# XiaoshuiHuang/IMFNet

Hardware: AMD Instinct MI355X
Metric: descriptors/sec (32-D) on 3DMatch fragments (higher is better)
Workload: dtype f32 (bf16x3)

## Files before the change

### imfnet_amd/_lib.py

```python
import ctypes as C
import os

_HERE = os.path.dirname(os.path.abspath(__file__))
LIB_PATH = os.environ.get("IMF_LIB") or os.path.join(_HERE, "libimfnet_hip.so")

TILE_ROWS = 64
MASK_WORDS = 4
MAX_KVOL = 125
MAX_BATCH = 8
FLAG_RANGE = 32
XYZ_F32_QUOTIENT = 2
TAG_LABEL, TAG_REGS, TAG_WAVE8, TAG_WAVE4, TAG_HEAD, TAG_HALF, TAG_U48, TAG_OCC = 1, 2, 4, 8, 16, 64, 128, 256


class ImfError(RuntimeError):
    pass


class ConvArgs(C.Structure):
    _fields_ = [
        ("in_a", C.c_void_p), ("in_b", C.c_void_p),
        ("c_a", C.c_int32), ("c_b", C.c_int32),
        ("w_packed", C.c_void_p),
        ("kvol", C.c_int32), ("cout", C.c_int32),
        ("tile_rows", C.c_void_p), ("nbr", C.c_void_p),
        ("tile_mask", C.c_void_p),
        ("n_slots", C.c_int64), ("n_out", C.c_int64),
        ("scale", C.c_void_p), ("shift", C.c_void_p), ("residual", C.c_void_p),
        ("relu", C.c_int32), ("l2norm", C.c_int32),
        ("out", C.c_void_p),
        ("split_k", C.c_int32), ("variant", C.c_int32),
        ("workspace", C.c_void_p), ("workspace_bytes", C.c_size_t),
        ("ev_begin", C.c_void_p), ("ev_end", C.c_void_p),
        ("n_out_dev", C.c_void_p), ("slots_extra", C.c_int32),
        ("kernel_tag", C.c_int32), ("dyn_err", C.c_void_p), ("geglu", C.c_int32), ("operand_format", C.c_int32),
    ]


class HeadArgs(C.Structure):
    _fields_ = [
        ("in_a", C.c_void_p), ("in_b", C.c_void_p), ("c_a", C.c_int32), ("c_b", C.c_int32),
        ("w1_packed", C.c_void_p), ("scale1", C.c_void_p), ("shift1", C.c_void_p),
        ("relu1", C.c_int32), ("c_mid", C.c_int32),
        ("w2_packed", C.c_void_p), ("scale2", C.c_void_p), ("shift2", C.c_void_p),
        ("l2norm", C.c_int32), ("c_out", C.c_int32),
        ("n", C.c_int64), ("n_dev", C.c_void_p), ("out", C.c_void_p), ("flags", C.c_void_p),
        ("ev_begin", C.c_void_p), ("ev_end", C.c_void_p), ("a_split", C.c_int32), ("variant", C.c_int32),
    ]


class LevelDesc(C.Structure):
    _fields_ = [("coords", C.c_void_p), ("table", C.c_void_p),
                ("capacity", C.c_int64), ("first_idx", C.c_void_p), ("cap_rows", C.c_int64),
                ("tensor_stride", C.c_int32)]


class FusionWeights(C.Structure):
    _fields_ = [(n, C.c_void_p) for n in ("ln1_g", "ln1_b", "wq_p", "wo_p", "bo", "ln2_g", "ln2_b", "w1_p", "b1",
                                          "w2_p", "b2", "w1_f32", "w2_f32")]


class NetConv(C.Structure):
    _fields_ = [("w_packed", C.c_void_p), ("kvol", C.c_int32), ("cin", C.c_int32), ("cout", C.c_int32),
                ("scale", C.c_void_p), ("shift", C.c_void_p), ("relu", C.c_int32), ("l2norm", C.c_int32),
                ("variant", C.c_int32)]


class ResunetDesc(C.Structure):
    _fields_ = [("channels", C.c_int32 * 5), ("tr_channels", C.c_int32 * 5), ("in_channels", C.c_int32),
                ("out_channels", C.c_int32), ("first_ksize", C.c_int32), ("small_first", C.c_int32),
                ("conv", NetConv * 23), ("first_kernel", C.c_void_p), ("first_scale", C.c_void_p),
                ("first_shift", C.c_void_p), ("fusion", FusionWeights), ("fusion_scale", C.c_float),
                ("first_kernel_image", C.c_void_p)]


class ImageDesc(C.Structure):
    _fields_ = [("stem_w", C.c_void_p), ("stem_scale", C.c_void_p), ("stem_shift", C.c_void_p),
                ("conv", NetConv * 15), ("ln_g", C.c_void_p), ("ln_b", C.c_void_p), ("kv_w", C.c_void_p),
                ("variant", C.c_int32)]


class ImageTable(C.Structure):
    _fields_ = [("tile_rows", C.c_void_p), ("nbr", C.c_void_p), ("tile_mask", C.c_void_p), ("n_slots", C.c_int64),
                ("n_out", C.c_int64), ("kvol", C.c_int32)]


IMAGE_TRAIN_TABLES = ("t4", "t48", "t48T", "td", "tdT", "t8")


class ImageTrainTables(C.Structure):
    _fields_ = [(n, ImageTable) for n in IMAGE_TRAIN_TABLES]


class NetTrace(C.Structure):
    _fields_ = [("ev_begin", C.c_void_p), ("ev_end", C.c_void_p), ("nbr", C.c_void_p), ("kvol", C.c_int32),
                ("cin", C.c_int32), ("cout", C.c_int32), ("split", C.c_int32), ("n_slots", C.c_int64),
                ("n_out", C.c_int64), ("launched", C.c_int32), ("level", C.c_int32), ("slots_extra", C.c_int32),
                ("kernel_tag", C.c_int32)]


class ResunetIO(C.Structure):
    _fields_ = [("level", LevelDesc * 4), ("n", C.c_int64 * 4), ("bbox", C.c_void_p), ("x", C.c_void_p),
                ("x_all_ones", C.c_int32), ("n_items", C.c_int32), ("item_row0", C.c_int64 * MAX_BATCH),
                ("item_rows", C.c_int64 * MAX_BATCH), ("kt_packed", C.c_void_p * MAX_BATCH),
                ("v_packed", C.c_void_p * MAX_BATCH),
                ("n_tokens", C.c_int32), ("tokens_padded", C.c_int32), ("image_ready", C.c_void_p),
                ("fusion_done", C.c_void_p), ("int_arena", C.c_void_p), ("int_arena_bytes", C.c_size_t),
                ("float_arena", C.c_void_p), ("float_arena_bytes", C.c_size_t), ("out", C.c_void_p),
                ("events", C.c_void_p * 16), ("side_stream", C.c_void_p), ("main_stream", C.c_void_p),
                ("trace", C.POINTER(NetTrace)), ("dyn", C.c_int32), ("meta", C.c_void_p),
                ("bitgrid_words", C.c_size_t), ("pyramid", C.c_void_p), ("flags", C.c_void_p),
                ("fp32_buffers", C.c_int32)]


DYN_WORDS = 16
META_WORDS = 64


class FragmentCaps(C.Structure):
    _fields_ = [("n_points", C.c_int64), ("rows", C.c_int64 * 4), ("n_items", C.c_int32), ("img_h", C.c_int32),
                ("img_w", C.c_int32), ("bitgrid_words", C.c_size_t)]


class FragmentIO(C.Structure):
    _fields_ = [("xyz", C.c_void_p), ("xyz_is_f64", C.c_int32), ("voxel_size", C.c_double), ("dyn", C.c_void_p),
                ("image", C.c_void_p), ("meta", C.c_void_p), ("pyramid_arena", C.c_void_p),
                ("pyramid_arena_bytes", C.c_size_t), ("image_ws", C.c_void_p), ("image_ws_bytes", C.c_size_t),
                ("kt_packed", C.c_void_p), ("v_packed", C.c_void_p), ("tokens_padded", C.c_int32),
                ("int_arena", C.c_void_p), ("int_arena_bytes", C.c_size_t), ("float_arena", C.c_void_p),
                ("float_arena_bytes", C.c_size_t), ("out", C.c_void_p), ("events", C.c_void_p * 16),
                ("main_stream", C.c_void_p), ("side_stream", C.c_void_p), ("image_stream", C.c_void_p),
                ("trace", C.POINTER(NetTrace)), ("levels", LevelDesc * 4), ("serialize", C.c_int32),
                ("fp32_buffers", C.c_int32), ("head_on_side", C.c_int32), ("gpu_idle_hint", C.c_int32),
                ("inputs_event", C.c_void_p), ("reuse_event", C.c_void_p)]


class TsdfParams(C.Structure):
    _fields_ = [("fx", C.c_double), ("fy", C.c_double), ("cx", C.c_double), ("cy", C.c_double),
                ("voxel_length", C.c_double), ("sdf_trunc", C.c_double), ("depth_scale", C.c_double),
                ("depth_trunc", C.c_double), ("lattice_offset", C.c_double), ("height", C.c_int32), ("width", C.c_int32)]


class OverlapIndex(C.Structure):
    _fields_ = [("table", C.c_void_p), ("capacity", C.c_int64), ("xyz", C.c_void_p), ("idx", C.c_void_p),
                ("cells", C.c_void_p), ("chunks", C.c_void_p), ("meta", C.c_void_p), ("n", C.c_int64), ("cell", C.c_double)]


class Job(C.Structure):
    _fields_ = [("net", C.POINTER(ResunetDesc)), ("img", C.POINTER(ImageDesc)), ("caps", C.POINTER(FragmentCaps)),
                ("io", C.POINTER(FragmentIO)), ("host_in", C.c_void_p), ("dev_in", C.c_void_p), ("in_bytes", C.c_size_t),
                ("dev_out", C.c_void_p), ("host_out", C.c_void_p), ("out_bytes", C.c_size_t), ("sel", C.c_void_p),
                ("sel_offset", C.c_size_t), ("out_offset", C.c_size_t), ("out_row_bytes", C.c_int32),
                ("defer_download", C.c_int32)]


PIPELINE_SDMA_COPIES = 1

_P, _I, _L, _D, _Z = C.c_void_p, C.c_int, C.c_int64, C.c_double, C.c_size_t

SIGNATURES = {
    "imf_version": (_I, []),
    "imf_last_error": (C.c_char_p, []),
    "imf_spconv_wgrad_workspace_bytes": (_Z, [_L, _I, _I, _I]),
    "imf_spconv_wgrad": (_I, [_P, _I, _P, _I, _P, _P, _L, _L, _I, _P, _P, _Z, _P]),
    "imf_bn_train_chunk_rows": (_I, []),
    "imf_bn_train_workspace_bytes": (_Z, [_L, _I]),
    "imf_bn_train_forward": (_I, [_P, _L, _I, _P, _P, _D, _P, _I, _P, _P, _D, _P, _P, _P, _Z, _P]),
    "imf_bn_train_backward": (_I, [_P, _P, _P, _I, _P, _P, _L, _I, _P, _P, _P, _P, _P, _Z, _P]),
    "imf_hc_loss_workspace_bytes": (_Z, [_L, _L, _I, _L, _L, _L, _L]),
    "imf_hc_loss_forward": (_I, [_P, _L, _P, _L, _I, _P, _L, _P, _L, _P, _L, _P, _L, _D, _D, _P, _P, _P, _P, _P, _P, _P,
                                 _Z, _P]),
    "imf_hc_loss_backward": (_I, [_P, _L, _P, _L, _I, _P, _L, _P, _L, _P, _L, _P, _L, _D, _D, _P, _P, _P, _P, _P, _P, _P,
                                  _P, _P, _Z, _P]),
    "imf_fusion_train_chunk_rows": (_I, []),
    "imf_fusion_train_saved_bytes": (_Z, [_L, _I, _I]),
    "imf_fusion_train_workspace_bytes": (_Z, [_L, _I, _I]),
    "imf_fusion_train_forward": (_I, [_P, _L, _P, _I, _P, _I, _I, _I, _I, _I, C.POINTER(C.c_void_p), _P, _P, _Z, _P, _P]),
    "imf_fusion_train_backward": (_I, [_P, _P, _L, _P, _I, _P, _I, _I, _I, _I, _I, C.POINTER(C.c_void_p), _P, _Z, _P, _P,
                                       C.POINTER(C.c_void_p), _P, _P, _Z, _P]),
    "imf_dam_heat": (_I, [_P, _L, _P, _P, _I, _I, _P, _I, _I, _P, _P, _P, _P, _P]),
    "imf_ply_vertex_count": (_L, [C.c_char_p]),
    "imf_ply_read_points": (_L, [C.c_char_p, _P, _L]),
    "imf_png_info": (_I, [C.c_char_p, C.POINTER(C.c_int), C.POINTER(C.c_int), C.POINTER(C.c_int)]),
    "imf_png_read_f32": (_I, [C.c_char_p, _P, _L, C.POINTER(C.c_int), C.POINTER(C.c_int), C.POINTER(C.c_int)]),
    "imf_png_read_u16": (_I, [C.c_char_p, _P, _L, C.POINTER(C.c_int), C.POINTER(C.c_int)]),
    "imf_ply_write_points": (_I, [C.c_char_p, _P, _L]),
    "imf_ply_write_points_rgb": (_I, [C.c_char_p, _P, _P, _L]),
    "imf_jpeg_info": (_I, [C.c_char_p, C.POINTER(C.c_int), C.POINTER(C.c_int), C.POINTER(C.c_int)]),
    "imf_jpeg_read_u8": (_I, [C.c_char_p, _P, _L, C.POINTER(C.c_int), C.POINTER(C.c_int), C.POINTER(C.c_int)]),
    "imf_resize_bilinear_f32": (_I, [_P, _I, _I, _I, _P, _I, _I, _I]),
    "imf_npz_write": (_I, [C.c_char_p, _I, C.POINTER(C.c_char_p), C.POINTER(C.c_char_p), C.POINTER(C.c_int32),
                           C.POINTER(C.c_int64), C.POINTER(C.c_void_p), _I]),
    "imf_npz_write_mt": (_I, [C.c_char_p, _I, C.POINTER(C.c_char_p), C.POINTER(C.c_char_p), C.POINTER(C.c_int32),
                              C.POINTER(C.c_int64), C.POINTER(C.c_void_p), _I, _I]),
    "imf_stream_create": (_P, []),
    "imf_stream_destroy": (None, [_P]),
    "imf_event_create": (_P, []),
    "imf_event_destroy": (None, [_P]),
    "imf_event_record": (_I, [_P, _P]),
    "imf_event_elapsed_ms": (C.c_float, [_P, _P]),
    "imf_nn_workspace_bytes": (_Z, [_L, _L]),
    "imf_nn_search": (_I, [_P, _L, _P, _L, _I, _P, _P, _P, _Z, _P]),
    "imf_mutual_inliers": (_I, [_P, _L, _P, _L, _P, _P, _P, _D, _P, _P, _P]),
    "imf_keypoint_workspace_bytes": (_Z, [_L, _L]),
    "imf_select_keypoints": (_I, [_P, _L, _P, _L, _D, _P, _P, _P, _Z, _P]),
    "imf_resunet_int_arena_bytes": (_Z, [C.POINTER(ResunetDesc), C.POINTER(C.c_int64), _P]),
    "imf_resunet_float_arena_bytes": (_Z, [C.POINTER(ResunetDesc), C.POINTER(C.c_int64)]),
    "imf_resunet_conv_kernel_tag": (_I, [_I, _I, _I, _I, _I, _I]),
    "imf_resunet_forward": (_I, [C.POINTER(ResunetDesc), C.POINTER(ResunetIO)]),
    "imf_resunet_int_arena_bytes_cap": (_Z, [C.POINTER(ResunetDesc), C.POINTER(C.c_int64), _Z]),
    "imf_resunet_float_arena_bytes_cap": (_Z, [C.POINTER(ResunetDesc), C.POINTER(C.c_int64)]),
    "imf_fragment_pyramid_bytes": (_Z, [C.POINTER(FragmentCaps)]),
    "imf_fragment_forward": (_I, [C.POINTER(ResunetDesc), C.POINTER(ImageDesc), C.POINTER(FragmentCaps),
                                  C.POINTER(FragmentIO)]),
    "imf_pipeline_create": (_P, [_P, _I, _I]),
    "imf_pipeline_destroy": (None, [_P]),
    "imf_pipeline_submit": (_I, [_P, C.POINTER(Job)]),
    "imf_pipeline_wait": (_I, [_P, _I, C.POINTER(C.c_float)]),
    "imf_host_narrow_points": (_I, [_P, _L, _P]),
    "imf_graph_begin_capture": (_I, [_P]),
    "imf_graph_end_capture": (_I, [_P, C.POINTER(C.c_void_p), C.POINTER(C.c_int)]),
    "imf_graph_abort_capture": (_I, [_P]),
    "imf_graph_launch": (_I, [_P, _P]),
    "imf_graph_destroy": (None, [_P]),
    "imf_pyramid_arena_bytes_caps": (_Z, [_L, _I, C.POINTER(C.c_int64)]),
    "imf_pyramid_build_dyn": (_I, [_P, _I, _P, _L, C.POINTER(C.c_int64), _D, _I, _P, _Z, _P, C.POINTER(LevelDesc), _P]),
    "imf_rulebook_conv_dyn": (_I, [_P, _L, _P, _L, _P, _I, _I, _P, _P, _P, _P]),
    "imf_rulebook_transpose_dyn": (_I, [_P, _L, _P, _L, _P, _I, _I, _P, _P, _P, _L, _P, _P]),
    "imf_conv_first_bitgrid_dyn": (_I, [_P, _L, _P, _P, _P, _I, _P, _Z, _P, _I, _P, _P, _I, _P, _P]),
    "imf_fusion_workspace_bytes_cap": (_Z, [_L]),
    "imf_fusion_attention_dyn": (_I, [_P, _L, _P, _P, _I, _P, C.POINTER(C.c_void_p), C.POINTER(C.c_void_p), _I, _I,
                                      C.POINTER(FusionWeights), C.c_float, _P, _P, _Z, _P]),
    "imf_ransac_workspace_bytes": (_Z, [_I]),
    "imf_ransac_registration": (_I, [_P, _L, _P, _L, _P, _I, _D, _D, _I, C.c_uint64, _P, _P, _P, _P, _Z, _P]),
    "imf_gather_points": (_I, [_P, _I, _P, _P, _L, _P, _P]),
    "imf_icp_workspace_bytes": (_Z, [_L, _L]),
    "imf_icp_point_to_point": (_I, [_P, _L, _P, _L, _D, _P, _I, _P, _P, _P, _P, _Z, _P]),
    "imf_radius_count_workspace_bytes": (_Z, [_L]),
    "imf_radius_count": (_I, [_P, _L, _P, _L, _P, _D, _P, _P, _P, _P, _Z, _P]),
    "imf_radius_pairs_workspace_bytes": (_Z, [_L, _L]),
    "imf_radius_pairs": (_I, [_P, _L, _P, _L, _P, _D, _P, _P, _L, _P, _P, _P, _Z, _P]),
    "imf_robust_transform_workspace_bytes": (_Z, [_L]),
    "imf_robust_transform": (_I, [_P, _P, _P, _L, _P, _P, _P, _Z, _P]),
    "imf_tsdf_allocate_workspace_bytes": (_Z, [_L]),
    "imf_tsdf_allocate": (_I, [_P, _I, _P, C.POINTER(TsdfParams), _I, _P, _L, _P, _L, _P, _P, _Z, _P]),
    "imf_tsdf_integrate": (_I, [_P, _I, _P, C.POINTER(TsdfParams), _P, _P, _L, _P, _P]),
    "imf_tsdf_extract_workspace_bytes": (_Z, [_L]),
    "imf_tsdf_extract": (_I, [_P, _P, _P, _L, _P, _L, C.POINTER(TsdfParams), _P, _L, _P, _P, _Z, _P]),
    "imf_overlap_index_bytes": (_Z, [_L]),
    "imf_overlap_index_workspace_bytes": (_Z, [_L]),
    "imf_overlap_index_build": (_I, [_P, _L, _D, _P, _Z, C.POINTER(OverlapIndex), _P, _Z, _P]),
    "imf_overlap_bound": (_I, [_P, _P, _I, _L, _P, _P]),
    "imf_overlap_pair": (_I, [C.POINTER(OverlapIndex), C.POINTER(OverlapIndex), C.c_float, _L, _P, _P]),
    "imf_overlap_emit_workspace_bytes": (_Z, [_L]),
    "imf_overlap_emit": (_I, [_P, _L, _P, _P, _P, _Z, _P]),
    "imf_hash_capacity": (_L, [_L]),
    "imf_unique_workspace_bytes": (_Z, [_L]),
    "imf_voxelize": (_I, [_P, _I, _L, _D, _I, _P, _P, _P, _P, _L, _P, _P, _P]),
    "imf_downsample": (_I, [_P, _P, _L, _I, _P, _P, _P, _L, _P, _P]),
    "imf_pyramid_arena_bytes": (_Z, [_L, _I]),
    "imf_pyramid_build": (_I, [_P, _I, _L, _D, _I, _I, _P, _Z, _P, C.POINTER(LevelDesc), _P]),
    "imf_pyramid_build_batched": (_I, [_P, _I, _L, _D, C.POINTER(C.c_int64), _I, _I, _P, _Z, _P,
                                       C.POINTER(LevelDesc), _P]),
    "imf_rulebook_slots": (_L, [_L]),
    "imf_rulebook_conv": (_I, [_P, _L, _P, _L, _I, _I, _P, _P, _P, _P]),
    "imf_rulebook_sorted_workspace_bytes": (C.c_size_t, [_L]),
    "imf_rulebook_sort_by_occupancy": (_I, [_P, _I, _L, _L, _P, _P, _P, _P, _P, C.c_size_t, _P]),
    "imf_resunet_sorted_maps": (_I, [_I]),
    "imf_resunet_sorted_maps_n": (_I, [_I, _I]),
    "imf_rulebook_transpose_slots": (_L, [_L]),
    "imf_rulebook_transpose": (_I, [_P, _L, _P, _L, _I, _I, _P, _P, _P, _L, _P, _P]),
    "imf_packed_weight_floats": (_L, [_I, _I, _I]),
    "imf_packed_weight_floats_split16": (_L, [_I, _I, _I]),
    "imf_pack_weights": (_I, [_P, _I, _I, _I, _P, _P]),
    "imf_first_kernel_image_floats": (_L, [_I, _I]),
    "imf_pack_first_kernel": (_I, [_P, _I, _I, _P, _P]),
    "imf_pack_weights_split16": (_I, [_P, _I, _I, _I, _P, _P]),
    "imf_packed_weight_floats_bf16x3": (_L, [_I, _I, _I]),
    "imf_pack_weights_bf16x3": (_I, [_P, _I, _I, _I, _P, _P]),
    "imf_spconv_auto_split": (_I, [_L, _I, _I]),
    "imf_spconv_workspace_bytes": (_Z, [_L, _I, _I]),
    "imf_spconv_fwd": (_I, [C.POINTER(ConvArgs), _P]),
    "imf_pointwise_head": (_I, [C.POINTER(HeadArgs), _P]),
    "imf_spconv_small_cin": (_I, [_P, _I, _P, _I, _I, _P, _L, _L, _P, _P, _I, _P, _P]),
    "imf_fusion_workspace_bytes": (_Z, [_L]),
    "imf_fusion_attention_batched": (_I, [_P, _I, C.POINTER(C.c_int64), C.POINTER(C.c_int64), C.POINTER(C.c_void_p),
                                          C.POINTER(C.c_void_p), _I, _I, C.POINTER(FusionWeights), C.c_float, _P, _P,
                                          _Z, _P]),
    "imf_fusion_attention": (_I, [_P, _L, _P, _P, _I, _I, C.POINTER(FusionWeights), C.c_float, _P, _P, _Z, _P]),
    "imf_fusion_attention_batched_v": (_I, [_P, _I, C.POINTER(C.c_int64), C.POINTER(C.c_int64), C.POINTER(C.c_void_p),
                                            C.POINTER(C.c_void_p), _I, _I, C.POINTER(FusionWeights), C.c_float, _P, _P,
                                            _Z, _P, _I, _P]),
    "imf_image_workspace_bytes": (_Z, [_I, _I, _I]),
    "imf_image_tokens": (_I, [_I, _I]),
    "imf_image_tables_build": (_I, [_I, _I, _I, _P, _Z, _P]),
    "imf_image_branch": (_I, [C.POINTER(ImageDesc), _P, _I, _I, _I, _P, _Z, _P, _P, _P, _I, _P, _P]),
    "imf_image_train_tables_bytes": (_Z, [_I, _I, _I]),
    "imf_image_train_tables_build": (_I, [_I, _I, _I, _P, _Z, C.POINTER(ImageTrainTables), _P]),
    "imf_image_im2col7": (_I, [_P, _I, _I, _I, _P, _P]),
    "imf_image_maxpool_forward": (_I, [_P, _I, _I, _I, _I, _P, _P, _P]),
    "imf_image_maxpool_backward": (_I, [_P, _P, _I, _I, _I, _I, _P, _P]),
    "imf_conv_first_bitgrid_flags": (_I, [_P, _L, _P, _I, _P, _Z, _P, _I, _P, _P, _I, _P, _P, _P]),
    "imf_fusion_attention_batched_flags": (_I, [_P, _I, C.POINTER(C.c_int64), C.POINTER(C.c_int64), C.POINTER(C.c_void_p),
                                                C.POINTER(C.c_void_p), _I, _I, C.POINTER(FusionWeights), C.c_float, _P, _P,
                                                _Z, _P, _P]),
    "imf_bitgrid_words": (_Z, [_P, _I]),
    "imf_conv_first_bitgrid": (_I, [_P, _L, _P, _I, _P, _Z, _P, _I, _P, _P, _I, _P, _P]),
    "imf_conv_first_fused": (_I, [_P, _L, _P, _L, _I, _I, _P, _I, _P, _I, _P, _P, _I, _P, _P]),
}

_lib = None


def lib():
    global _lib
    if _lib is None:
        if not os.path.exists(LIB_PATH):
            raise ImfError(
                f"{LIB_PATH} not found: build it with `python -c 'import __graft_entry__ as g; g.build()'` "
                "or `make -C imfnet_amd/csrc`.  imfnet_amd has no CPU fallback.")
        handle = C.CDLL(LIB_PATH)
        for name, (res, args) in SIGNATURES.items():
            fn = getattr(handle, name)
            fn.restype, fn.argtypes = res, args
        _lib = handle
    return _lib


def check(rc, what):
    if rc != 0:
        msg = lib().imf_last_error().decode("utf-8", "replace")
        raise ImfError(f"{what} failed (rc={rc}): {msg}")
```

### imfnet_amd/csrc/rulebook_sort.hip

```cpp
#include <hip/hip_runtime.h>
#include <cstring>

#include "common.h"

namespace imf {
namespace {

constexpr int kWindowShift = 14;
constexpr int kWindow = 1 << kWindowShift;
constexpr int kSortThreads = 1024, kSortWaves = kSortThreads / 64, kPerThread = kWindow / kSortThreads;
constexpr int kDigitBits = 6, kDigits = 1 << kDigitBits, kPasses = 3, kKeyBits = kDigitBits * kPasses;
constexpr int kMaxGroups = kWindow / kSortWaves / 64;

__device__ __forceinline__ constexpr int key_bit_of_offset(int k) {
  constexpr int edges[12] = {1, 3, 5, 7, 9, 11, 15, 17, 19, 21, 23, 25};
  constexpr int faces[6] = {4, 10, 12, 14, 16, 22};
  for (int i = 0; i < 12; ++i)
    if (edges[i] == k) return 17 - i;
  for (int i = 0; i < 6; ++i)
    if (faces[i] == k) return 5 - i;
  return -1;
}

__device__ __forceinline__ unsigned gray_inverse18(unsigned r) {
  r ^= r >> 1;
  r ^= r >> 2;
  r ^= r >> 4;
  r ^= r >> 8;
  r ^= r >> 16;
  return r & 0x3FFFFu;
}

template <int KVOL>
__global__ void __launch_bounds__(256)
k_rbs_keys(const int32_t *__restrict__ nbr, int kvol_rt, long long n_slots, long long n_out, const int32_t *__restrict__ n_dev,
           unsigned *__restrict__ keys) {
  const long long s = (long long)blockIdx.x * blockDim.x + threadIdx.x;
  long long n = n_out;
  if (n_dev) n = *n_dev < n ? *n_dev : n;
  if (s >= n || s >= n_slots) return;
  const int kvol = KVOL ? KVOL : kvol_rt;
  unsigned r = 0u;
  if (KVOL == 27) {
#pragma unroll
    for (int k = 0; k < 27; ++k) {
      const int bit = key_bit_of_offset(k);
      if (bit >= 0) r |= (nbr[(long long)k * n_slots + s] >= 0 ? 1u : 0u) << bit;
    }
  } else {
    for (int k = 0; k < kvol && k < kKeyBits; ++k) r |= (nbr[(long long)k * n_slots + s] >= 0 ? 1u : 0u) << k;
  }
  keys[s] = gray_inverse18(r);
}

constexpr size_t kSortLdsBytes = sizeof(unsigned) * (2 * kWindow + kSortWaves * kDigits + 2 * kDigits);
#if defined(__HIP_DEVICE_COMPILE__) && !defined(__gfx950__)
#error "k_rbs_window_sort keeps a 16 384-slot window in 132 KiB of LDS: build for gfx950 (160 KiB per workgroup)"
#endif
static_assert(kSortLdsBytes <= 160 * 1024, "k_rbs_window_sort: static LDS exceeds gfx950's 160 KiB per workgroup");

__global__ void __launch_bounds__(kSortThreads)
k_rbs_window_sort(const unsigned *__restrict__ keys, long long n_slots, long long n_out,
                  const int32_t *__restrict__ n_dev, int32_t *__restrict__ perm) {
  __shared__ unsigned val0[kWindow], val1[kWindow];
  __shared__ unsigned hist[kSortWaves * kDigits], dtot[kDigits], doff[kDigits];
  const int tid = threadIdx.x, lane = tid & 63, wave = tid >> 6;
  const long long wbase = (long long)blockIdx.x * kWindow;
  long long n = n_out;
  if (n_dev) n = *n_dev < n ? *n_dev : n;
  const int n_win = (int)((n_slots - wbase) < kWindow ? (n_slots - wbase) : kWindow);
  const int n_valid = (int)(n - wbase < 0 ? 0 : (n - wbase < n_win ? n - wbase : n_win));
  const int groups = ((n_valid + kSortWaves - 1) / kSortWaves + 63) / 64;
  const int per_wave = groups * 64, n_pos = per_wave * kSortWaves;

#pragma unroll 4
  for (int i = 0; i < kPerThread; ++i) {
    const int loc = tid + kSortThreads * i;
    if (loc < n_pos) val0[loc] = ((loc < n_valid ? keys[wbase + loc] : (1u << kKeyBits) - 1u) << kWindowShift) | (unsigned)loc;
  }
  __syncthreads();

  unsigned *src = val0, *dst = val1;
  unsigned *const myhist = hist + wave * kDigits;
  const int chunk = wave * per_wave;
  const unsigned long long below = (1ull << lane) - 1ull;
#pragma unroll 1
  for (int pass = 0; pass < kPasses; ++pass) {
    const int shift = kWindowShift + kDigitBits * pass;
    for (int d = tid; d < kSortWaves * kDigits; d += kSortThreads) hist[d] = 0u;
    __syncthreads();
    unsigned word[kMaxGroups], info[kMaxGroups];
#pragma unroll
    for (int g = 0; g < kMaxGroups; ++g) {
      if (g < groups) {
        const unsigned v = src[chunk + 64 * g + lane];
        const unsigned d = (v >> shift) & (kDigits - 1);
        unsigned long long same = ~0ull;
#pragma unroll
        for (int b = 0; b < kDigitBits; ++b) {
          const bool bit = (d >> b) & 1u;
          const unsigned long long bal = __ballot(bit);
          same &= bit ? bal : ~bal;
        }
        const unsigned rank = (unsigned)__builtin_popcountll(same & below), cnt = (unsigned)__builtin_popcountll(same);
        if (rank == 0) atomicAdd(&myhist[d], cnt);
        word[g] = v;
        info[g] = d | (rank << 6) | ((cnt - 1u) << 12);
      }
    }
    __syncthreads();
    if (tid < kDigits) {
      unsigned run = 0u;
#pragma unroll
      for (int w = 0; w < kSortWaves; ++w) {
        const unsigned c = hist[w * kDigits + tid];
        hist[w * kDigits + tid] = run;
        run += c;
      }
      unsigned incl = run;
#pragma unroll
      for (int o = 1; o < 64; o <<= 1) {
        const unsigned up = __shfl_up(incl, o, 64);
        if (tid >= o) incl += up;
      }
      doff[tid] = incl - run;
    }
    __syncthreads();
#pragma unroll
    for (int g = 0; g < kMaxGroups; ++g) {
      if (g < groups) {
        const unsigned d = info[g] & 63u, rank = (info[g] >> 6) & 63u, last = info[g] >> 12;
        const unsigned base = myhist[d];
        if (rank == last) myhist[d] = base + last + 1u;
        dst[base + doff[d] + rank] = word[g];
      }
    }
    __syncthreads();
    unsigned *const t = src;
    src = dst;
    dst = t;
  }

  for (int loc = tid; loc < n_win; loc += kSortThreads)
    perm[wbase + loc] = loc < n_valid ? (int32_t)(wbase + (src[loc] & (kWindow - 1))) : -1;
  (void)dtot;
}

constexpr long long kGatherInFlightSlots = 256 * 4 * 64;

template <int KVOL>
__global__ void __launch_bounds__(256)
k_rbs_gather(const int32_t *__restrict__ nbr, int kvol, long long n_slots, long long n_out, const int32_t *__restrict__ n_dev,
             const int32_t *__restrict__ perm, int32_t *__restrict__ tile_rows, int32_t *__restrict__ nbr_out,
             uint32_t *__restrict__ tile_mask) {
  const long long s = (long long)blockIdx.x * blockDim.x + threadIdx.x;
  if (s >= n_slots) return;
  long long n = n_out;
  if (n_dev) n = *n_dev < n ? *n_dev : n;
  const int r = perm[s];
  const bool valid = r >= 0 && r < n;
  tile_rows[s] = valid ? r : -1;
  uint32_t m = 0u;
  if (KVOL == 27) {
    const int32_t *src = nbr + (valid ? r : 0);
    int v[27];
#pragma unroll
    for (int k = 0; k < 27; ++k) v[k] = src[(long long)k * n_slots];
#pragma unroll
    for (int k = 0; k < 27; ++k) {
      const int w = valid ? v[k] : -1;
      nbr_out[(long long)k * n_slots + s] = w;
      if (__ballot(w >= 0) != 0ull) m |= 1u << k;
    }
  } else {
    for (int k = 0; k < kvol; ++k) {
      const int v = valid ? nbr[(long long)k * n_slots + r] : -1;
      nbr_out[(long long)k * n_slots + s] = v;
      if (__ballot(v >= 0) != 0ull) m |= 1u << k;
    }
  }
  if ((threadIdx.x & 63) == 0) {
    uint32_t *t = tile_mask + (s >> 6) * IMF_MASK_WORDS;
    t[0] = m;
    for (int w = 1; w < IMF_MASK_WORDS; ++w) t[w] = 0u;
  }
}

}
}

using namespace imf;

extern "C" {

size_t imf_rulebook_sorted_workspace_bytes(int64_t n_slots) {
  if (n_slots <= 0) return 0;
  return 2 * ((((size_t)n_slots + 63) / 64 * 64) * 4 + 255) / 256 * 256;
}

int imf_rulebook_sort_by_occupancy(const int32_t *nbr_in, int kvol, int64_t n_slots, int64_t n_out, const int32_t *n_out_dev,
                                   int32_t *tile_rows, int32_t *nbr_out, uint32_t *tile_mask, void *workspace,
                                   size_t workspace_bytes, void *stream) {
  IMF_REQUIRE(nbr_in && tile_rows && nbr_out && tile_mask && workspace, "imf_rulebook_sort_by_occupancy: null pointer");
  IMF_REQUIRE(kvol >= 1 && kvol <= 27, "imf_rulebook_sort_by_occupancy: kvol=%d (1 .. 27)", kvol);
  IMF_REQUIRE(n_slots > 0 && n_slots % IMF_TILE_ROWS == 0 && n_out > 0 && n_out <= n_slots && n_slots < (1ll << 31),
              "imf_rulebook_sort_by_occupancy: n_slots=%lld n_out=%lld (whole tiles)", (long long)n_slots, (long long)n_out);
  IMF_REQUIRE(workspace_bytes >= imf_rulebook_sorted_workspace_bytes(n_slots), "imf_rulebook_sort_by_occupancy: workspace %zu < %zu bytes",
              workspace_bytes, imf_rulebook_sorted_workspace_bytes(n_slots));
  IMF_REQUIRE(nbr_in != nbr_out, "imf_rulebook_sort_by_occupancy: in place");
  hipStream_t st = (hipStream_t)stream;
  int32_t *perm = (int32_t *)workspace;
  const unsigned windows = (unsigned)((n_slots + kWindow - 1) / kWindow);
  const unsigned blocks = (unsigned)((n_slots + 255) / 256);
  unsigned *keys = (unsigned *)(perm + (((size_t)n_slots + 63) / 64 * 64));
  if (kvol == 27) k_rbs_keys<27><<<blocks, 256, 0, st>>>(nbr_in, kvol, n_slots, n_out, n_out_dev, keys);
  else            k_rbs_keys<0><<<blocks, 256, 0, st>>>(nbr_in, kvol, n_slots, n_out, n_out_dev, keys);
  IMF_CHECK_LAUNCH("k_rbs_keys");
  k_rbs_window_sort<<<windows, kSortThreads, 0, st>>>(keys, n_slots, n_out, n_out_dev, perm);
  IMF_CHECK_LAUNCH("k_rbs_window_sort");
  if (kvol == 27 && n_slots <= kGatherInFlightSlots) k_rbs_gather<27><<<blocks, 256, 0, st>>>(nbr_in, kvol, n_slots, n_out, n_out_dev, perm, tile_rows, nbr_out, tile_mask);
  else            k_rbs_gather<0><<<blocks, 256, 0, st>>>(nbr_in, kvol, n_slots, n_out, n_out_dev, perm, tile_rows, nbr_out, tile_mask);
  IMF_CHECK_LAUNCH("k_rbs_gather");
  return IMF_OK;
}

}
```

### include/imfnet_hip.h

```cpp
#ifndef IMFNET_HIP_H
#define IMFNET_HIP_H

#include <stddef.h>
#include <stdint.h>

#ifdef __cplusplus
extern "C" {
#endif

#define IMF_OK            0
#define IMF_EINVAL       -1
#define IMF_ELAUNCH      -2
#define IMF_EUNSUPPORTED -3

#define IMF_TILE_ROWS    64
#define IMF_MAX_KVOL     125
#define IMF_MAX_BATCH    8
#define IMF_MASK_WORDS   4
#define IMF_XYZ_F32_QUOTIENT 2

int imf_version(void);
const char *imf_last_error(void);

typedef struct imf_slot {
  uint64_t key;
  int32_t val;
  int32_t pad;
} imf_slot;
int64_t imf_hash_capacity(int64_t n);

size_t imf_unique_workspace_bytes(int64_t n);

int imf_voxelize(const void *xyz, int xyz_is_f64, int64_t n, double voxel_size, int batch_index,
                 int32_t *coords, int32_t *first_idx, int32_t *m_out,
                 imf_slot *table, int64_t capacity,
                 void *workspace, int32_t *err_out, void *stream);

int imf_downsample(const int32_t *coords_in, const int32_t *n_in_dev, int64_t n_in_max,
                   int out_stride,
                   int32_t *coords_out, int32_t *m_out,
                   imf_slot *table, int64_t capacity,
                   void *workspace, void *stream);

int imf_gather_points(const void *xyz, int xyz_is_f64, const int32_t *first_idx, const int32_t *m_dev, int64_t m_cap,
                      double *out, void *stream);

typedef struct imf_level {
  int32_t *coords;
  imf_slot *table;
  int64_t capacity;
  int32_t *first_idx;
  int64_t cap_rows;
  int32_t tensor_stride;
} imf_level;

size_t imf_pyramid_arena_bytes(int64_t n_points, int n_levels);
int imf_pyramid_build(const void *xyz, int xyz_is_f64, int64_t n, double voxel_size, int batch_index,
                      int n_levels, void *arena, size_t arena_bytes, int32_t *meta,
                      imf_level *levels_out , void *stream);
int imf_pyramid_build_batched(const void *xyz, int xyz_is_f64, int64_t n, double voxel_size,
                              const int64_t *item_starts , int n_items, int n_levels, void *arena,
                              size_t arena_bytes, int32_t *meta, imf_level *levels_out, void *stream);

size_t imf_pyramid_arena_bytes_caps(int64_t n_points_cap, int n_levels, const int64_t *row_caps );
int imf_pyramid_build_dyn(const void *xyz, int xyz_is_f64, const int32_t *dyn, int64_t n_points_cap,
                          const int64_t *row_caps , double voxel_size, int n_levels, void *arena,
                          size_t arena_bytes, int32_t *meta, imf_level *levels_out , void *stream);


int64_t imf_rulebook_slots(int64_t n_out);

int imf_rulebook_conv(const imf_slot *in_table, int64_t in_capacity,
                      const int32_t *out_coords, int64_t n_out, int ts_in, int ksize,
                      int32_t *tile_rows, int32_t *nbr, uint32_t *tile_mask, void *stream);

size_t imf_rulebook_sorted_workspace_bytes(int64_t n_slots);
int imf_rulebook_sort_by_occupancy(const int32_t *nbr_in, int kvol, int64_t n_slots, int64_t n_out, const int32_t *n_out_dev,
                                   int32_t *tile_rows, int32_t *nbr_out, uint32_t *tile_mask, void *workspace,
                                   size_t workspace_bytes, void *stream);

int imf_rulebook_conv_dyn(const imf_slot *in_table, int64_t in_capacity,
                          const int32_t *out_coords, int64_t n_out_cap, const int32_t *n_out_dev, int ts_in,
                          int ksize, int32_t *tile_rows, int32_t *nbr, uint32_t *tile_mask, void *stream);

int64_t imf_rulebook_transpose_slots(int64_t n_fine);

int imf_rulebook_transpose(const imf_slot *coarse_table, int64_t coarse_capacity,
                           const int32_t *fine_coords, int64_t n_fine, int ts_fine, int ksize,
                           int32_t *tile_rows, int32_t *nbr, uint32_t *tile_mask,
                           int64_t n_slots, int32_t *counters, void *stream);

int imf_rulebook_transpose_dyn(const imf_slot *coarse_table, int64_t coarse_capacity,
                               const int32_t *fine_coords, int64_t n_fine_cap, const int32_t *n_fine_dev, int ts_fine,
                               int ksize, int32_t *tile_rows, int32_t *nbr, uint32_t *tile_mask, int64_t n_slots,
                               int32_t *counters, void *stream);


int64_t imf_packed_weight_floats(int kvol, int cin, int cout);

int imf_pack_weights(const float *w, int kvol, int cin, int cout, float *packed, void *stream);
int64_t imf_packed_weight_floats_split16(int kvol, int cin, int cout);
int imf_pack_weights_split16(const float *w, int kvol, int cin, int cout, float *packed, void *stream);
int64_t imf_packed_weight_floats_bf16x3(int kvol, int cin, int cout);
int imf_pack_weights_bf16x3(const float *w, int kvol, int cin, int cout, float *packed, void *stream);

typedef struct imf_conv_args {
  const float *in_a;
  const float *in_b;
  int32_t c_a, c_b;
  const float *w_packed;
  int32_t kvol, cout;
  const int32_t *tile_rows;
  const int32_t *nbr;
  const uint32_t *tile_mask;
  int64_t n_slots, n_out;
  const float *scale;
  const float *shift;
  const float *residual;
  int32_t relu;
  int32_t l2norm;
  float *out;
  int32_t split_k;
  int32_t variant;
  void *workspace;
  size_t workspace_bytes;
  void *ev_begin, *ev_end;
  const int32_t *n_out_dev;
  int32_t slots_extra;
  int32_t kernel_tag;
  int32_t *dyn_err;
  int32_t geglu;
  int32_t operand_format;
} imf_conv_args;
#define IMF_TAG_LABEL   1
#define IMF_TAG_REGS    2
#define IMF_TAG_WAVE8   4
#define IMF_TAG_WAVE4   8
#define IMF_TAG_HEAD   16
#define IMF_TAG_HALF   64
#define IMF_TAG_U48   128
#define IMF_TAG_OCC   256

#define IMF_FMT_A_SPLIT   1
#define IMF_FMT_RES_SPLIT 2
#define IMF_FMT_OUT_SPLIT 4

#define IMF_FLAG_COORD_RANGE  1
#define IMF_FLAG_CAPACITY     2
#define IMF_FLAG_BITGRID      4
#define IMF_FLAG_EMPTY_ITEM   8
#define IMF_FLAG_RANGE       32

int imf_spconv_auto_split(int64_t n_slots, int cout, int kvol);
size_t imf_spconv_workspace_bytes(int64_t n_slots, int cout, int split);

int imf_spconv_fwd(const imf_conv_args *args , void *stream);

typedef struct imf_head_args {
  const float *in_a;
  const float *in_b;
  int32_t c_a, c_b;
  const float *w1_packed;
  const float *scale1, *shift1;
  int32_t relu1, c_mid;
  const float *w2_packed;
  const float *scale2, *shift2;
  int32_t l2norm, c_out;
  int64_t n;
  const int32_t *n_dev;
  float *out;
  int32_t *flags;
  void *ev_begin, *ev_end;
  int32_t a_split;
  int32_t variant;
} imf_head_args;
int imf_pointwise_head(const imf_head_args *args , void *stream);

int imf_spconv_small_cin(const float *in, int cin, const float *w, int kvol, int cout,
                         const int32_t *nbr, int64_t n_slots, int64_t n_out,
                         const float *scale, const float *shift, int relu,
                         float *out, void *stream);

int imf_conv_first_fused(const imf_slot *table, int64_t capacity,
                         const int32_t *coords, int64_t n, int ts, int ksize, const float *in, int cin,
                         const float *w , int cout,
                         const float *scale, const float *shift, int relu, float *out, void *stream);

size_t imf_bitgrid_words(const int32_t *bbox , int ksize);
int imf_conv_first_bitgrid(const int32_t *coords, int64_t n, const int32_t *bbox , int ksize,
                           uint32_t *grid, size_t grid_words, const float *w ,
                           int cout, const float *scale, const float *shift, int relu, float *out,
                           void *stream);

int imf_conv_first_bitgrid_flags(const int32_t *coords, int64_t n, const int32_t *bbox , int ksize,
                                 uint32_t *grid, size_t grid_words, const float *w, int cout, const float *scale,
                                 const float *shift, int relu, float *out, int32_t *flags, void *stream);
int imf_conv_first_bitgrid_dyn(const int32_t *coords, int64_t n_cap, const int32_t *n_dev, const int32_t *bbox_dev,
                               int32_t *err, int ksize, uint32_t *grid, size_t grid_words, const float *w, int cout,
                               const float *scale, const float *shift, int relu, float *out, void *stream);

typedef struct imf_fusion_weights {
  const float *ln1_g, *ln1_b, *wq_p, *wo_p, *bo, *ln2_g, *ln2_b, *w1_p, *b1, *w2_p, *b2;
  const float *w1_f32, *w2_f32;
} imf_fusion_weights;
size_t imf_fusion_workspace_bytes(int64_t n);
int imf_fusion_attention(const float *x, int64_t n, const float *kt_packed, const float *v_packed,
                         int n_tokens, int tokens_padded, const imf_fusion_weights *w ,
                         float scale, float *out, void *workspace, size_t workspace_bytes, void *stream);
int imf_fusion_attention_batched(const float *x, int n_items, const int64_t *item_row0, const int64_t *item_rows,
                                 const float *const *kt_packed, const float *const *v_packed, int n_tokens,
                                 int tokens_padded, const imf_fusion_weights *w , float scale, float *out,
                                 void *workspace, size_t workspace_bytes, void *stream);
int imf_fusion_attention_batched_v(const float *x, int n_items, const int64_t *item_row0, const int64_t *item_rows,
                                   const float *const *kt_packed, const float *const *v_packed, int n_tokens,
                                   int tokens_padded, const imf_fusion_weights *w , float scale, float *out,
                                   void *workspace, size_t workspace_bytes, int32_t *flags, int variant, void *stream);

typedef struct imf_net_conv {
  const float *w_packed;
  int32_t kvol, cin, cout;
  const float *scale, *shift;
  int32_t relu, l2norm, variant;
} imf_net_conv;

typedef struct imf_image_desc {
  const float *stem_w, *stem_scale, *stem_shift;
  imf_net_conv conv[15];
  const float *ln_g, *ln_b;
  const float *kv_w;
  int32_t variant;
} imf_image_desc;

size_t imf_image_workspace_bytes(int B, int H, int W);
int imf_image_tokens(int H, int W);
int imf_image_tables_build(int B, int H, int W, void *workspace, size_t workspace_bytes, void *stream);
int imf_image_branch(const imf_image_desc *net , const float *image, int B, int H, int W,
                     void *workspace, size_t workspace_bytes, float *feat_out, float *kt_packed,
                     float *v_packed, int tokens_padded, int32_t *flags ,
                     void *stream);

typedef struct imf_image_table {
  int32_t *tile_rows, *nbr;
  uint32_t *tile_mask;
  int64_t n_slots, n_out;
  int32_t kvol;
} imf_image_table;
typedef struct imf_image_train_tables {
  imf_image_table t4, t48, t48T, td, tdT, t8;
} imf_image_train_tables;
size_t imf_image_train_tables_bytes(int B, int H, int W);
int imf_image_train_tables_build(int B, int H, int W, void *storage, size_t storage_bytes,
                                 imf_image_train_tables *out , void *stream);
int imf_image_im2col7(const float *image_nchw, int B, int H, int W, float *out, void *stream);
int imf_image_maxpool_forward(const float *in, int B, int Hin, int Win, int C, float *out, uint8_t *tap, void *stream);
int imf_image_maxpool_backward(const float *dout, const uint8_t *tap, int B, int Hin, int Win, int C, float *din,
                               void *stream);

int imf_fusion_attention_batched_flags(const float *x, int n_items, const int64_t *item_row0, const int64_t *item_rows,
                                       const float *const *kt_packed, const float *const *v_packed, int n_tokens,
                                       int tokens_padded, const imf_fusion_weights *w , float scale,
                                       float *out, void *workspace, size_t workspace_bytes, int32_t *flags, void *stream);
size_t imf_fusion_workspace_bytes_cap(int64_t n_cap);
int imf_fusion_attention_dyn(const float *x, int64_t n_cap, const int32_t *n_dev, const int32_t *item_starts_dev,
                             int n_items, int32_t *err, const float *const *kt_packed, const float *const *v_packed,
                             int n_tokens, int tokens_padded, const imf_fusion_weights *w , float scale,
                             float *out, void *workspace, size_t workspace_bytes, void *stream);


typedef struct imf_resunet_desc {
  int32_t channels[5], tr_channels[5];
  int32_t in_channels, out_channels, first_ksize;
  int32_t small_first;
  imf_net_conv conv[23];
  const float *first_kernel, *first_scale, *first_shift;
  imf_fusion_weights fusion;
  float fusion_scale;
  const float *first_kernel_image;
} imf_resunet_desc;
int64_t imf_first_kernel_image_floats(int kvol, int cout);
int imf_pack_first_kernel(const float *w , int kvol, int cout, float *image, void *stream);

typedef struct imf_net_trace {
  void *ev_begin, *ev_end;
  const int32_t *nbr;
  int32_t kvol, cin, cout, split;
  int64_t n_slots, n_out;
  int32_t launched;
  int32_t level, slots_extra;
  int32_t kernel_tag;
} imf_net_trace;

int imf_resunet_conv_kernel_tag(int level, int kvol, int cin, int cout, int variant, int n_items);
int imf_resunet_sorted_maps(int variant);
int imf_resunet_sorted_maps_n(int variant, int n_items);

typedef struct imf_resunet_io {
  imf_level level[4];
  int64_t n[4];
  const int32_t *bbox;
  const float *x;
  int32_t x_all_ones;
  int32_t n_items;
  int64_t item_row0[IMF_MAX_BATCH];
  int64_t item_rows[IMF_MAX_BATCH];
  const float *kt_packed[IMF_MAX_BATCH], *v_packed[IMF_MAX_BATCH];
  int32_t n_tokens, tokens_padded;
  void *image_ready;
  void *fusion_done;
  void *int_arena;  size_t int_arena_bytes;
  void *float_arena; size_t float_arena_bytes;
  float *out;
  void *events[16];
  void *side_stream, *main_stream;
  imf_net_trace *trace;
  int32_t dyn;
  const int32_t *meta;
  size_t bitgrid_words;
  const void *pyramid;
  int32_t *flags;
  int32_t fp32_buffers;
} imf_resunet_io;

size_t imf_resunet_int_arena_bytes(const imf_resunet_desc *net, const int64_t *n ,
                                   const int32_t *bbox );
size_t imf_resunet_float_arena_bytes(const imf_resunet_desc *net, const int64_t *n );
int imf_resunet_forward(const imf_resunet_desc *net , const imf_resunet_io *io );
size_t imf_resunet_int_arena_bytes_cap(const imf_resunet_desc *net, const int64_t *row_caps , size_t bitgrid_words);
size_t imf_resunet_float_arena_bytes_cap(const imf_resunet_desc *net, const int64_t *row_caps );

#define IMF_DYN_WORDS  16
#define IMF_META_WORDS 64
typedef struct imf_fragment_caps {
  int64_t n_points;
  int64_t rows[4];
  int32_t n_items, img_h, img_w;
  size_t bitgrid_words;
} imf_fragment_caps;

typedef struct imf_fragment_io {
  const void *xyz; int32_t xyz_is_f64;
  double voxel_size;
  const int32_t *dyn;
  const float *image;
  int32_t *meta;
  void *pyramid_arena; size_t pyramid_arena_bytes;
  void *image_ws; size_t image_ws_bytes;
  float *kt_packed, *v_packed; int32_t tokens_padded;
  void *int_arena; size_t int_arena_bytes;
  void *float_arena; size_t float_arena_bytes;
  float *out;
  void *events[16];
  void *main_stream, *side_stream, *image_stream;
  imf_net_trace *trace;
  imf_level levels[4];
  int32_t serialize;
  int32_t fp32_buffers;
  int32_t head_on_side;
  int32_t gpu_idle_hint;
  void *inputs_event, *reuse_event;
} imf_fragment_io;

size_t imf_fragment_pyramid_bytes(const imf_fragment_caps *caps);
int imf_fragment_forward(const imf_resunet_desc *net , const imf_image_desc *img ,
                         const imf_fragment_caps *caps, imf_fragment_io *io);

typedef struct imf_job {
  const imf_resunet_desc *net;
  const imf_image_desc *img;
  const imf_fragment_caps *caps;
  imf_fragment_io *io;
  const void *host_in; void *dev_in; size_t in_bytes;
  const void *dev_out; void *host_out; size_t out_bytes;
  double *sel;
  size_t sel_offset;
  size_t out_offset; int32_t out_row_bytes;
  int32_t defer_download;
} imf_job;
#define IMF_PIPELINE_SDMA_COPIES 1
void *imf_pipeline_create(void *main_stream, int depth , int flags);
// ... 176 lines not shown
```

Measured before the change: 92.61 million.

## Rework rulebook window sort to two 9-bit passes and add windowed gather

Changes the per-window LDS radix sort from three 6-bit passes to two 9-bit passes and keeps keys in registers, so a single LDS buffer replaces the ping-pong pair. Histogram offsets now come from atomic returns broadcast within a wave, and the kernel is templated on group count. For large slot counts, a new per-window, per-offset gather kernel stages each neighbor slice in LDS, and tile_mask zeroing is folded into the key kernel. This cuts sort passes and improves gather locality, at the cost of more complex code and new correctness risk in the mask and ranking logic.

```diff
diff --git a/imfnet_amd/_lib.py b/imfnet_amd/_lib.py
--- a/imfnet_amd/_lib.py
+++ b/imfnet_amd/_lib.py
@@ -265,6 +265,7 @@
     "imf_rulebook_slots": (_L, [_L]),
     "imf_rulebook_conv": (_I, [_P, _L, _P, _L, _I, _I, _P, _P, _P, _P]),
     "imf_rulebook_sorted_workspace_bytes": (C.c_size_t, [_L]),
+    "imf_rulebook_sort_lds_bytes": (C.c_size_t, []),
     "imf_rulebook_sort_by_occupancy": (_I, [_P, _I, _L, _L, _P, _P, _P, _P, _P, C.c_size_t, _P]),
     "imf_resunet_sorted_maps": (_I, [_I]),
     "imf_resunet_sorted_maps_n": (_I, [_I, _I]),
diff --git a/imfnet_amd/csrc/rulebook_sort.hip b/imfnet_amd/csrc/rulebook_sort.hip
--- a/imfnet_amd/csrc/rulebook_sort.hip
+++ b/imfnet_amd/csrc/rulebook_sort.hip
@@ -8,9 +8,10 @@
 
 constexpr int kWindowShift = 14;
 constexpr int kWindow = 1 << kWindowShift;
-constexpr int kSortThreads = 1024, kSortWaves = kSortThreads / 64, kPerThread = kWindow / kSortThreads;
-constexpr int kDigitBits = 6, kDigits = 1 << kDigitBits, kPasses = 3, kKeyBits = kDigitBits * kPasses;
+constexpr int kSortThreads = 1024, kSortWaves = kSortThreads / 64;
+constexpr int kDigitBits = 9, kDigits = 1 << kDigitBits, kPasses = 2, kKeyBits = kDigitBits * kPasses;
 constexpr int kMaxGroups = kWindow / kSortWaves / 64;
+constexpr int kScanWaves = kDigits / 64;
 
 __device__ __forceinline__ constexpr int key_bit_of_offset(int k) {
   constexpr int edges[12] = {1, 3, 5, 7, 9, 11, 15, 17, 19, 21, 23, 25};
@@ -34,8 +35,9 @@
 template <int KVOL>
 __global__ void __launch_bounds__(256)
 k_rbs_keys(const int32_t *__restrict__ nbr, int kvol_rt, long long n_slots, long long n_out, const int32_t *__restrict__ n_dev,
-           unsigned *__restrict__ keys) {
+           unsigned *__restrict__ keys, uint32_t *__restrict__ zero_mask) {
   const long long s = (long long)blockIdx.x * blockDim.x + threadIdx.x;
+  if (zero_mask && s < n_slots / IMF_TILE_ROWS * IMF_MASK_WORDS) zero_mask[s] = 0u;
   long long n = n_out;
   if (n_dev) n = *n_dev < n ? *n_dev : n;
   if (s >= n || s >= n_slots) return;
@@ -53,97 +55,127 @@
   keys[s] = gray_inverse18(r);
 }
 
-constexpr size_t kSortLdsBytes = sizeof(unsigned) * (2 * kWindow + kSortWaves * kDigits + 2 * kDigits);
+constexpr size_t kSortLdsBytes = sizeof(unsigned) * (kWindow + kSortWaves * kDigits + kScanWaves);
 #if defined(__HIP_DEVICE_COMPILE__) && !defined(__gfx950__)
-#error "k_rbs_window_sort keeps a 16 384-slot window in 132 KiB of LDS: build for gfx950 (160 KiB per workgroup)"
+#error "k_rbs_window_sort keeps a 16 384-slot window in 96 KiB of LDS: build for gfx950 (160 KiB per workgroup)"
 #endif
 static_assert(kSortLdsBytes <= 160 * 1024, "k_rbs_window_sort: static LDS exceeds gfx950's 160 KiB per workgroup");
+
+__device__ __forceinline__ unsigned long long same_digit_lanes(unsigned d) {
+  unsigned lo = ~0u, hi = ~0u;
+#pragma unroll
+  for (int b = 0; b < kDigitBits; ++b) {
+    const unsigned m = (unsigned)((int)(d << (31 - b)) >> 31);
+    const unsigned long long bal = __ballot(m != 0u);
+    lo &= ~((unsigned)bal ^ m);
+    hi &= ~((unsigned)(bal >> 32) ^ m);
+  }
+  return ((unsigned long long)hi << 32) | lo;
+}
+
+template <int G>
+__device__ __forceinline__ void sort_window(const unsigned *__restrict__ keys, long long wbase, int n_valid, unsigned *val, unsigned *hist,
+                                            unsigned *wtot) {
+  const int tid = threadIdx.x, lane = tid & 63, wave = tid >> 6;
+  const int chunk = wave * (G * 64);
+  unsigned *const myhist = hist + wave * kDigits;
+
+  unsigned word[G];
+#pragma unroll
+  for (int g = 0; g < G; ++g) {
+    const int loc = chunk + 64 * g + lane;
+    word[g] = ((loc < n_valid ? keys[wbase + loc] : (1u << kKeyBits) - 1u) << kWindowShift) | (unsigned)loc;
+  }
+
+#pragma unroll
+  for (int pass = 0; pass < kPasses; ++pass) {
+    const int shift = kWindowShift + kDigitBits * pass;
+    if (pass > 0) {
+#pragma unroll
+      for (int g = 0; g < G; ++g) word[g] = val[chunk + 64 * g + lane];
+    }
+    for (int d = tid; d < kSortWaves * kDigits; d += kSortThreads) hist[d] = 0u;
+    __syncthreads();
+
+    unsigned info[G], seen[G], first[G];
+#pragma unroll
+    for (int g = 0; g < G + 2; ++g) {
+      unsigned d = 0u, rank = 1u, cnt = 0u;
+      if (g < G) {
+        d = (word[g] >> shift) & (kDigits - 1);
+        const unsigned long long same = same_digit_lanes(d);
+        rank = __builtin_amdgcn_mbcnt_hi((unsigned)(same >> 32), __builtin_amdgcn_mbcnt_lo((unsigned)same, 0u));
+        cnt = (unsigned)__builtin_popcountll(same);
+        info[g] = d | (rank << kDigitBits) | ((unsigned)__builtin_ctzll(same) << 15);
+      }
+      if (g >= 2) info[g - 2] = (info[g - 2] & (kDigits - 1)) | ((first[g - 2] + ((info[g - 2] >> kDigitBits) & 63u)) << kDigitBits);
+      if (g >= 1 && g <= G) first[g - 1] = __shfl(seen[g - 1], (int)(info[g - 1] >> 15), 64);
+      if (g < G) {
+        seen[g] = 0u;
+        if (rank == 0) seen[g] = atomicAdd(&myhist[d], cnt);
+        __builtin_amdgcn_fence(__ATOMIC_ACQ_REL, "wavefront");
+        __builtin_amdgcn_wave_barrier();
+      }
+    }
+    __syncthreads();
+
+    unsigned before[kSortWaves], run = 0u, incl = 0u;
+    if (tid < kDigits) {
+#pragma unroll
+      for (int w = 0; w < kSortWaves; ++w) before[w] = hist[w * kDigits + tid];
+#pragma unroll
+      for (int w = 0; w < kSortWaves; ++w) {
+        const unsigned c = before[w];
+        before[w] = run;
+        run += c;
+      }
+      incl = run;
+#pragma unroll
+      for (int o = 1; o < 64; o <<= 1) {
+        const unsigned up = __shfl_up(incl, o, 64);
+        if (lane >= o) incl += up;
+      }
+      if (lane == 63) wtot[wave] = incl;
+    }
+    __syncthreads();
+    if (tid < kDigits) {
+      unsigned base = incl - run;
+#pragma unroll
+      for (int w = 0; w < kScanWaves - 1; ++w) base += w < wave ? wtot[w] : 0u;
+#pragma unroll
+      for (int w = 0; w < kSortWaves; ++w) hist[w * kDigits + tid] = base + before[w];
+    }
+    __syncthreads();
+
+    unsigned pos[G];
+#pragma unroll
+    for (int g = 0; g < G; ++g) pos[g] = myhist[info[g] & (kDigits - 1)] + (info[g] >> kDigitBits);
+#pragma unroll
+    for (int g = 0; g < G; ++g) val[pos[g]] = word[g];
+    __syncthreads();
+  }
+}
 
 __global__ void __launch_bounds__(kSortThreads)
 k_rbs_window_sort(const unsigned *__restrict__ keys, long long n_slots, long long n_out,
                   const int32_t *__restrict__ n_dev, int32_t *__restrict__ perm) {
-  __shared__ unsigned val0[kWindow], val1[kWindow];
-  __shared__ unsigned hist[kSortWaves * kDigits], dtot[kDigits], doff[kDigits];
-  const int tid = threadIdx.x, lane = tid & 63, wave = tid >> 6;
+  __shared__ unsigned val[kWindow];
+  __shared__ unsigned hist[kSortWaves * kDigits];
+  __shared__ unsigned wtot[kScanWaves];
+  const int tid = threadIdx.x;
   const long long wbase = (long long)blockIdx.x * kWindow;
   long long n = n_out;
   if (n_dev) n = *n_dev < n ? *n_dev : n;
   const int n_win = (int)((n_slots - wbase) < kWindow ? (n_slots - wbase) : kWindow);
   const int n_valid = (int)(n - wbase < 0 ? 0 : (n - wbase < n_win ? n - wbase : n_win));
   const int groups = ((n_valid + kSortWaves - 1) / kSortWaves + 63) / 64;
-  const int per_wave = groups * 64, n_pos = per_wave * kSortWaves;
-
-#pragma unroll 4
-  for (int i = 0; i < kPerThread; ++i) {
-    const int loc = tid + kSortThreads * i;
-    if (loc < n_pos) val0[loc] = ((loc < n_valid ? keys[wbase + loc] : (1u << kKeyBits) - 1u) << kWindowShift) | (unsigned)loc;
-  }
-  __syncthreads();
-
-  unsigned *src = val0, *dst = val1;
-  unsigned *const myhist = hist + wave * kDigits;
-  const int chunk = wave * per_wave;
-  const unsigned long long below = (1ull << lane) - 1ull;
-#pragma unroll 1
-  for (int pass = 0; pass < kPasses; ++pass) {
-    const int shift = kWindowShift + kDigitBits * pass;
-    for (int d = tid; d < kSortWaves * kDigits; d += kSortThreads) hist[d] = 0u;
-    __syncthreads();
-    unsigned word[kMaxGroups], info[kMaxGroups];
-#pragma unroll
-    for (int g = 0; g < kMaxGroups; ++g) {
-      if (g < groups) {
-        const unsigned v = src[chunk + 64 * g + lane];
-        const unsigned d = (v >> shift) & (kDigits - 1);
-        unsigned long long same = ~0ull;
-#pragma unroll
-        for (int b = 0; b < kDigitBits; ++b) {
-          const bool bit = (d >> b) & 1u;
-          const unsigned long long bal = __ballot(bit);
-          same &= bit ? bal : ~bal;
-        }
-        const unsigned rank = (unsigned)__builtin_popcountll(same & below), cnt = (unsigned)__builtin_popcountll(same);
-        if (rank == 0) atomicAdd(&myhist[d], cnt);
-        word[g] = v;
-        info[g] = d | (rank << 6) | ((cnt - 1u) << 12);
-      }
-    }
-    __syncthreads();
-    if (tid < kDigits) {
-      unsigned run = 0u;
-#pragma unroll
-      for (int w = 0; w < kSortWaves; ++w) {
-        const unsigned c = hist[w * kDigits + tid];
-        hist[w * kDigits + tid] = run;
-        run += c;
-      }
-      unsigned incl = run;
-#pragma unroll
-      for (int o = 1; o < 64; o <<= 1) {
-        const unsigned up = __shfl_up(incl, o, 64);
-        if (tid >= o) incl += up;
-      }
-      doff[tid] = incl - run;
-    }
-    __syncthreads();
-#pragma unroll
-    for (int g = 0; g < kMaxGroups; ++g) {
-      if (g < groups) {
-        const unsigned d = info[g] & 63u, rank = (info[g] >> 6) & 63u, last = info[g] >> 12;
-        const unsigned base = myhist[d];
-        if (rank == last) myhist[d] = base + last + 1u;
-        dst[base + doff[d] + rank] = word[g];
-      }
-    }
-    __syncthreads();
-    unsigned *const t = src;
-    src = dst;
-    dst = t;
-  }
+  if (groups > 12)     sort_window<kMaxGroups>(keys, wbase, n_valid, val, hist, wtot);
+  else if (groups > 8) sort_window<12>(keys, wbase, n_valid, val, hist, wtot);
+  else if (groups > 4) sort_window<8>(keys, wbase, n_valid, val, hist, wtot);
+  else if (groups > 0) sort_window<4>(keys, wbase, n_valid, val, hist, wtot);
 
   for (int loc = tid; loc < n_win; loc += kSortThreads)
-    perm[wbase + loc] = loc < n_valid ? (int32_t)(wbase + (src[loc] & (kWindow - 1))) : -1;
-  (void)dtot;
+    perm[wbase + loc] = loc < n_valid ? (int32_t)(wbase + (val[loc] & (kWindow - 1))) : -1;
 }
 
 constexpr long long kGatherInFlightSlots = 256 * 4 * 64;
@@ -186,12 +218,51 @@
   }
 }
 
+__global__ void __launch_bounds__(kSortThreads)
+k_rbs_gather_window(const int32_t *__restrict__ nbr, int kvol, long long n_slots, long long n_out, const int32_t *__restrict__ n_dev,
+                    const int32_t *__restrict__ perm, int32_t *__restrict__ tile_rows, int32_t *__restrict__ nbr_out,
+                    uint32_t *__restrict__ tile_mask) {
+  __shared__ int32_t slice[kWindow];
+  const int tid = threadIdx.x;
+  const int k = blockIdx.x % kvol;
+  const long long wbase = (long long)(blockIdx.x / kvol) * kWindow;
+  long long n = n_out;
+  if (n_dev) n = *n_dev < n ? *n_dev : n;
+  const int n_win = (int)((n_slots - wbase) < kWindow ? (n_slots - wbase) : kWindow);
+  const int32_t *src = nbr + (long long)k * n_slots + wbase;
+  int32_t *dst = nbr_out + (long long)k * n_slots + wbase;
+  int r[kWindow / kSortThreads];
+#pragma unroll
+  for (int i = 0; i < kWindow / kSortThreads; ++i) {
+    const int loc = tid + kSortThreads * i;
+    r[i] = -1;
+    if (loc < n_win) {
+      r[i] = perm[wbase + loc];
+      slice[loc] = src[loc];
+    }
+  }
+  __syncthreads();
+#pragma unroll
+  for (int i = 0; i < kWindow / kSortThreads; ++i) {
+    const int loc = tid + kSortThreads * i;
+    if (loc < n_win) {
+      const bool valid = r[i] >= wbase && r[i] < n && r[i] < wbase + n_win;
+      const int v = valid ? slice[r[i] - wbase] : -1;
+      dst[loc] = v;
+      if (k == 0) tile_rows[wbase + loc] = valid ? r[i] : -1;
+      if (__ballot(v >= 0) != 0ull && (tid & 63) == 0) atomicOr(tile_mask + ((wbase + loc) >> 6) * IMF_MASK_WORDS, 1u << k);
+    }
+  }
+}
+
 }
 }
 
 using namespace imf;
 
 extern "C" {
+
+size_t imf_rulebook_sort_lds_bytes(void) { return kSortLdsBytes; }
 
 size_t imf_rulebook_sorted_workspace_bytes(int64_t n_slots) {
   if (n_slots <= 0) return 0;
@@ -213,12 +284,15 @@
   const unsigned windows = (unsigned)((n_slots + kWindow - 1) / kWindow);
   const unsigned blocks = (unsigned)((n_slots + 255) / 256);
   unsigned *keys = (unsigned *)(perm + (((size_t)n_slots + 63) / 64 * 64));
-  if (kvol == 27) k_rbs_keys<27><<<blocks, 256, 0, st>>>(nbr_in, kvol, n_slots, n_out, n_out_dev, keys);
-  else            k_rbs_keys<0><<<blocks, 256, 0, st>>>(nbr_in, kvol, n_slots, n_out, n_out_dev, keys);
+  const bool by_window = n_slots > kGatherInFlightSlots;
+  uint32_t *zero_mask = by_window ? tile_mask : nullptr;
+  if (kvol == 27) k_rbs_keys<27><<<blocks, 256, 0, st>>>(nbr_in, kvol, n_slots, n_out, n_out_dev, keys, zero_mask);
+  else            k_rbs_keys<0><<<blocks, 256, 0, st>>>(nbr_in, kvol, n_slots, n_out, n_out_dev, keys, zero_mask);
   IMF_CHECK_LAUNCH("k_rbs_keys");
   k_rbs_window_sort<<<windows, kSortThreads, 0, st>>>(keys, n_slots, n_out, n_out_dev, perm);
   IMF_CHECK_LAUNCH("k_rbs_window_sort");
-  if (kvol == 27 && n_slots <= kGatherInFlightSlots) k_rbs_gather<27><<<blocks, 256, 0, st>>>(nbr_in, kvol, n_slots, n_out, n_out_dev, perm, tile_rows, nbr_out, tile_mask);
+  if (by_window)  k_rbs_gather_window<<<windows * (unsigned)kvol, kSortThreads, 0, st>>>(nbr_in, kvol, n_slots, n_out, n_out_dev, perm, tile_rows, nbr_out, tile_mask);
+  else if (kvol == 27) k_rbs_gather<27><<<blocks, 256, 0, st>>>(nbr_in, kvol, n_slots, n_out, n_out_dev, perm, tile_rows, nbr_out, tile_mask);
   else            k_rbs_gather<0><<<blocks, 256, 0, st>>>(nbr_in, kvol, n_slots, n_out, n_out_dev, perm, tile_rows, nbr_out, tile_mask);
   IMF_CHECK_LAUNCH("k_rbs_gather");
   return IMF_OK;
diff --git a/include/imfnet_hip.h b/include/imfnet_hip.h
--- a/include/imfnet_hip.h
+++ b/include/imfnet_hip.h
@@ -75,6 +75,7 @@
                       int32_t *tile_rows, int32_t *nbr, uint32_t *tile_mask, void *stream);
 
 size_t imf_rulebook_sorted_workspace_bytes(int64_t n_slots);
+size_t imf_rulebook_sort_lds_bytes(void);
 int imf_rulebook_sort_by_occupancy(const int32_t *nbr_in, int kvol, int64_t n_slots, int64_t n_out, const int32_t *n_out_dev,
                                    int32_t *tile_rows, int32_t *nbr_out, uint32_t *tile_mask, void *workspace,
                                    size_t workspace_bytes, void *stream);
```

Measured after the change: 92.52 million (median of 2 runs). No clear change (-0.1%).
